# OSOceanAcoustics/echopype

Hardware: AMD Instinct MI355X
Metric: range-samples/sec through compute_Sv->compute_MVBS (higher is better)
Workload: dtype f64; 1 GPU; cfg5: EK60 CW 4x2000000x4096 in ping_time tiles, compute_Sv -> compute_MVBS(20s x 1m), Sv+MVBS out; tiles=8 x 250000 pings over 1 rank(s), route=compute_Sv -> compute_MVBS('1m','20s') per tile, collective=none at 1 rank, tile_streams=2

## Files before the change

### echopype_amd/csrc/fused_sv_mvbs.hip

```cpp
#include <hip/amd_detail/amd_hip_unsafe_atomics.h>

#include <cstdlib>
#include <type_traits>

#include "fast_math.h"
#include "sample_math.h"

namespace epa_fused {

constexpr int VEC = 4;
constexpr int kChunk = epa::kBlock * VEC;

struct Args {
  int P, S, n_tbins, n_rbins;
  double range_bin, inv_range_bin;
  double nspread, fill_value;
  unsigned guard, mask_range, skipna, closed_right;
  unsigned cnt_off, tab_off;
  unsigned long long* rmax_key;
  unsigned long long* rstat;
  int xcd_map;
  int flagged_only;
  const double* dscale;
  const double* doffset;
  void* depth_out;
};

__device__ __forceinline__ unsigned long long ordered_key(double v) {
  const unsigned long long b = __double_as_longlong(v);
  return (b >> 63) ? ~b : (b | 0x8000000000000000ull);
}

template <typename T>
__device__ __noinline__ T log10_slow(T x) {
  return epa::M<T>::log10(x);
}

template <typename T>
__device__ __forceinline__ void lds_add(T* p, T v) {
  unsafeAtomicAdd(p, v);
}

template <typename T>
struct Column {
  double sra;
  double blo, bhi;
  T nL;
  T acc_sum;
  int acc_rb;
  uint32_t acc_cnt;
  __device__ __forceinline__ void init() {
    sra = 0.0; blo = 1.0; bhi = 0.0; nL = epa::M<T>::nan(); acc_sum = (T)0; acc_rb = -1; acc_cnt = 0u;
  }
  __device__ __forceinline__ void flush(T* lsum, uint32_t* lcnt, uint32_t n_clean) {
    const uint32_t n = acc_cnt + n_clean;
    if (acc_rb >= 0 && n > 0u) {
      lds_add(lsum + acc_rb, acc_sum);
      atomicAdd(lcnt + acc_rb, n);
    }
  }
  __device__ __forceinline__ void rebin(double x, bool valid, double bin, double inv_bin, int n_rbins, T* lsum,
                                        uint32_t* lcnt, uint32_t n_clean) {
    const int rb = valid ? epa::range_bin_index(x, bin, inv_bin, n_rbins, false) : -1;
    if (rb != acc_rb) {
      flush(lsum, lcnt, n_clean);
      acc_rb = rb;
      acc_sum = (T)0;
      acc_cnt = 0u - n_clean;
    }
    blo = rb >= 0 ? (double)rb * bin : 1.0;
    bhi = rb >= 0 ? (double)(rb + 1) * bin : 0.0;
  }
};

__device__ __forceinline__ double lin_bins(double u, const double* __restrict__ tab) {
  constexpr double K256 = 85.04135922911648, Z = 0.0027076061740622863;
  constexpr double C1 = Z, C2 = Z * Z / 2.0, C3 = Z * Z * Z / 6.0;
  const double t = u * K256;
  const double m = __builtin_rint(t);
  const double r = fma(u, K256, -m);
  double p = fma(r, C3, C2);
  p = fma(p, r, C1);
  p = fma(p, r, 1.0);
  const int mi = __double2int_rz(m);
  return ldexp(p * tab[mi & 255], mi >> 8);
}
__device__ __forceinline__ float lin_bins(float u, const double*) { return ::exp10f(u * 0.1f); }

__device__ __forceinline__ double vmax_num(double a, double b) {
  double r;
  asm("v_max_f64 %0, %1, %2" : "=v"(r) : "v"(a), "v"(b));
  return r;
}
__device__ __forceinline__ float vmax_num(float a, float b) {
  float r;
  asm("v_max_f32 %0, %1, %2" : "=v"(r) : "v"(a), "v"(b));
  return r;
}
__device__ __forceinline__ double vmin_num(double a, double b) {
  double r;
  asm("v_min_f64 %0, %1, %2" : "=v"(r) : "v"(a), "v"(b));
  return r;
}

template <typename T, bool STATS>
__device__ __forceinline__ T process_sample(Column<T>& c, float raw, const epa::CoefRow& r, double r0v, T g, T a2,
                                            T A0v, T nL, T nspread, double bin, double inv_bin, int n_rbins,
                                            const double* tab, T* lsum, uint32_t* lcnt, double& xmax, double& xmin,
                                            unsigned& nnan, uint32_t n_clean) {
  const T NaN = epa::M<T>::nan();
  const double x = fma(c.sra, r.rb, r0v);
  if (STATS) {
    const double xq = fma((double)raw, 0.0, x);
    xmax = vmax_num(xmax, xq);
    xmin = vmin_num(xmin, xq);
    nnan += (unsigned)__builtin_popcountll(__ballot(raw != raw));
  }
  const double rtd = x - r.shift;
  const T rt = (T)rtd;
  const bool pos = rtd > 0.0;
  T s1 = fma(g, (T)raw, nL);
  if (pos & !(nL > -(T)__builtin_inf()))
    s1 = fma(g, (T)raw, nspread * (log10_slow<T>(rt) - log10_slow<T>((T)(r.ra * r.rb))));
  s1 = pos ? s1 : NaN;
  const T sv = s1 + fma(a2, rt, A0v);
  const T v = epa::lin_from_db_lean(sv, tab);
  const bool same = (x >= c.blo) & (x < c.bhi);
  if (!same) c.rebin(x, raw == raw, bin, inv_bin, n_rbins, lsum, lcnt, n_clean);
  c.acc_sum += vmax_num(v, (T)0);
  c.acc_cnt += v == v ? 1u : 0u;
  return sv;
}

template <typename T, bool STATS, bool WRITE_SV, int DEPTH>
__device__ __forceinline__ void process_pair(Column<T>& c0, Column<T>& c1, float2 in, bool clean, const epa::CoefRow& r,
                                             double r0v, T g, T a2, T A0v, T nL0, T nL1, T nspread, double bin,
                                             double inv_bin, int n_rbins, const double* tab, T* lsum, uint32_t* lcnt,
                                             T* __restrict__ sv_dst, double& xmax, double& xmin, unsigned& nnan,
                                             uint32_t n_clean, double& xfirst, double& xlast, T dsc, T dof,
                                             T* __restrict__ depth_dst, double sra0, double sra1) {
  const double e0 = fma(sra0, r.rb, r0v), e1 = fma(sra1, r.rb, r0v);
  const double rtd0 = e0 - r.shift, rtd1 = e1 - r.shift;
  T d0 = (T)0, d1 = (T)0;
  if (DEPTH) {
    d0 = epa::depth_of(dsc, dof, (T)e0);
    d1 = epa::depth_of(dsc, dof, (T)e1);
  }
  const double x0 = DEPTH ? (double)d0 : e0, x1 = DEPTH ? (double)d1 : e1;
  const T rt0 = (T)rtd0, rt1 = (T)rtd1;
  T s10 = fma(g, (T)in.x, nL0), s11 = fma(g, (T)in.y, nL1);
  if (!clean) {
    const T NaN = epa::M<T>::nan();
    const bool pos0 = rtd0 > 0.0, pos1 = rtd1 > 0.0;
    if (pos0 & !(nL0 > -(T)__builtin_inf()))
      s10 = fma(g, (T)in.x, nspread * (log10_slow<T>(rt0) - log10_slow<T>((T)(r.ra * r.rb))));
    if (pos1 & !(nL1 > -(T)__builtin_inf()))
      s11 = fma(g, (T)in.y, nspread * (log10_slow<T>(rt1) - log10_slow<T>((T)(r.ra * r.rb))));
    s10 = pos0 ? s10 : NaN;
    s11 = pos1 ? s11 : NaN;
    if (STATS) {
      const double xq0 = fma((double)in.x, 0.0, x0), xq1 = fma((double)in.y, 0.0, x1);
      xmax = vmax_num(vmax_num(xmax, xq0), xq1);
      xmin = vmin_num(vmin_num(xmin, xq0), xq1);
      nnan += (unsigned)__builtin_popcountll(__ballot(xq0 != xq0)) + (unsigned)__builtin_popcountll(__ballot(xq1 != xq1));
    }
    if (DEPTH == 2) {
      d0 = fma((T)in.x, (T)0, d0);
      d1 = fma((T)in.y, (T)0, d1);
    }
  }
  if (DEPTH == 2) epa::store_nt2(depth_dst, d0, d1);
  const T sv0 = s10 + fma(a2, rt0, A0v), sv1 = s11 + fma(a2, rt1, A0v);
  if (WRITE_SV) {
#ifndef EPA_PLAIN_STORES
    epa::store_nt2(sv_dst, sv0, sv1);
#else
    const T o[2] = {sv0, sv1};
    epa::store_vec<T, 2>(sv_dst, o);
#endif
  }
  T v0 = lin_bins(sv0, tab), v1 = lin_bins(sv1, tab);
  if (!clean) {
    if (__builtin_expect(__builtin_isinf(sv0), 0)) v0 = sv0 < (T)0 ? (T)0 : sv0;
    if (__builtin_expect(__builtin_isinf(sv1), 0)) v1 = sv1 < (T)0 ? (T)0 : sv1;
  }
  if (!((x0 >= c0.blo) & (x0 < c0.bhi))) c0.rebin(x0, in.x == in.x, bin, inv_bin, n_rbins, lsum, lcnt, n_clean);
  if (!((x1 >= c1.blo) & (x1 < c1.bhi))) c1.rebin(x1, in.y == in.y, bin, inv_bin, n_rbins, lsum, lcnt, n_clean);
  if (clean) {
    c0.acc_sum += v0;
    c1.acc_sum += v1;
  } else {
    c0.acc_sum += vmax_num(v0, (T)0);
    c1.acc_sum += vmax_num(v1, (T)0);
    c0.acc_cnt += v0 == v0 ? 1u : 0u;
    c1.acc_cnt += v1 == v1 ? 1u : 0u;
  }
  xfirst = x0;
  xlast = x1;
}

__device__ __forceinline__ bool not_finite(float x) { return __builtin_amdgcn_classf(x, 0x207); }

template <typename RawT>
struct PingLoad;
template <>
struct PingLoad<float> {
  float2 a, b;
  __device__ __forceinline__ PingLoad() : a(make_float2(0.f, 0.f)), b(make_float2(0.f, 0.f)) {}
  __device__ __forceinline__ void issue(const float* __restrict__ row, int sA, int sB, bool hasB, int, int) {
    a = *reinterpret_cast<const float2*>(row + sA);
    if (hasB) b = *reinterpret_cast<const float2*>(row + sB);
  }
  __device__ __forceinline__ void resolve(float2& A, float2& B, int, int, int, bool) const {
    A = a;
    B = b;
  }
};
template <>
struct PingLoad<int16_t> {
  unsigned a, b;
  __device__ __forceinline__ PingLoad() : a(0u), b(0u) {}
  __device__ __forceinline__ void issue(const int16_t* __restrict__ row, int sA, int sB, bool hasB, int, int) {
    a = *reinterpret_cast<const unsigned*>(row + sA);
    if (hasB) b = *reinterpret_cast<const unsigned*>(row + sB);
  }
  static __device__ __forceinline__ float2 unpack(unsigned w, int s, int n_valid) {
    constexpr float kIndex2Power = 0.011758984205624266f;
    const float nanv = __builtin_nanf("");
    const float x = (float)(short)(w & 0xffffu), y = (float)(short)(w >> 16);
    return make_float2(s < n_valid ? x * kIndex2Power : nanv, s + 1 < n_valid ? y * kIndex2Power : nanv);
  }
  static __device__ __forceinline__ float2 unpack_all(unsigned w) {
    constexpr float kIndex2Power = 0.011758984205624266f;
    return make_float2((float)(short)(w & 0xffffu) * kIndex2Power, (float)(short)(w >> 16) * kIndex2Power);
  }
  __device__ __forceinline__ void resolve(float2& A, float2& B, int sA, int sB, int nv, bool full) const {
    if (full) {
      A = unpack_all(a);
      B = unpack_all(b);
    } else {
      A = unpack(a, sA, nv);
      B = unpack(b, sB, nv);
    }
  }
};

#ifndef EPA_FUSED_MIN_WAVES
#define EPA_FUSED_MIN_WAVES 1
#endif
#ifndef EPA_FUSED_LEAN
#define EPA_FUSED_LEAN 1
#endif
__device__ __forceinline__ double uniform(double v) {
  return __hiloint2double(__builtin_amdgcn_readfirstlane(__double2hiint(v)), __builtin_amdgcn_readfirstlane(__double2loint(v)));
}

__device__ __forceinline__ bool finite_bits(double v) { return (__double2hiint(v) & 0x7ff00000) != 0x7ff00000; }

template <typename T, typename RawT, bool WRITE_SV, bool RMAX, int DEPTH>
__global__ __launch_bounds__(epa::kBlock, EPA_FUSED_MIN_WAVES > 4 ? EPA_FUSED_MIN_WAVES : 4) void fused_sv_mvbs_kernel(
    const RawT* __restrict__ raw, const int32_t* __restrict__ n_valid,
    const epa::CoefRow* __restrict__ coef,
    const int32_t* __restrict__ bin_start, T* __restrict__ sv_out, T* __restrict__ mvbs_out,
    T* __restrict__ sum_out, uint32_t* __restrict__ cnt_out, const double* __restrict__ dscale,
    const double* __restrict__ doffset, Args a) {
  extern __shared__ __attribute__((aligned(16))) unsigned char smem[];
  T* lsum = reinterpret_cast<T*>(smem);
  uint32_t* lcnt = reinterpret_cast<uint32_t*>(smem + a.cnt_off);
  const epa::MathTabs mt = epa::build_math_tabs(smem + a.tab_off);
  const double* tab = mt.exp2_tab;
  constexpr bool NL_LDS = RMAX || sizeof(T) == 8;
  __shared__ T col_nL[NL_LDS ? kChunk : 1];
  constexpr bool SRA_LDS = (RMAX || std::is_same<RawT, int16_t>::value) && sizeof(T) == 8;
  __shared__ double col_sra[SRA_LDS ? kChunk : 1];
  __shared__ unsigned long long wg_keys[2];
  __shared__ unsigned wg_nnan;
  if (RMAX && threadIdx.x == 0) {
    wg_keys[0] = 0ull;
    wg_keys[1] = ~0ull;
    wg_nnan = 0u;
  }

  const int c = blockIdx.y, tb = a.xcd_map ? epa::xcd_contiguous(blockIdx.x, a.n_tbins) : (int)blockIdx.x;
  const int S = a.S, n_rbins = a.n_rbins;
  const bool extra = tb == a.n_tbins;
  if (extra && !WRITE_SV) return;
  const int nseg = extra ? 2 : 1;
  for (int i = threadIdx.x; i < n_rbins; i += epa::kBlock) {
    lsum[i] = (T)0;
    lcnt[i] = 0u;
  }
  __syncthreads();

  const T nspread = (T)a.nspread;
  const double bin = a.range_bin, inv_bin = a.inv_range_bin;
  const epa::CoefRow* __restrict__ rowp0 = coef + (size_t)c * a.P;
  const RawT* __restrict__ raw_c = raw + (size_t)c * a.P * S;
  const int32_t* __restrict__ nv_c = n_valid ? n_valid + (size_t)c * a.P : nullptr;
  T* __restrict__ sv_c = WRITE_SV ? sv_out + (size_t)c * a.P * S : nullptr;
  T* __restrict__ dp_c = DEPTH == 2 ? reinterpret_cast<T*>(a.depth_out) + (size_t)c * a.P * S : nullptr;
  const double* __restrict__ dsc_c = DEPTH ? dscale + (size_t)c * a.P : nullptr;
  const double* __restrict__ dof_c = DEPTH ? doffset + (size_t)c * a.P : nullptr;
  const int wave = __builtin_amdgcn_readfirstlane((int)(threadIdx.x >> 6)), lane = threadIdx.x & 63;
  double xmax = -__builtin_inf(), xmin = __builtin_inf();
  unsigned nnan = 0u;

  for (int seg = 0; seg < nseg; ++seg) {
  const int pb = extra ? (seg == 0 ? 0 : bin_start[a.n_tbins]) : bin_start[tb];
  const int pe = extra ? (seg == 0 ? bin_start[0] : a.P) : bin_start[tb + 1];
  for (int chunk0 = 0; chunk0 < S; chunk0 += kChunk) {
    const int sA = chunk0 + wave * 256 + 2 * lane;
    const int sB = sA + 128;
    if (sA >= S) continue;
    const bool hasB = sB < S;
    Column<T> col[VEC];
#pragma unroll
    for (int j = 0; j < VEC; ++j) col[j].init();
    const int eA = wave * 256 + 2 * lane;
    if (NL_LDS) {
      col_nL[eA] = col_nL[eA + 1] = col_nL[eA + 128] = col_nL[eA + 129] = epa::M<T>::nan();
    }
    long long dcur = 0x7ff8dead00000001ll, racur = 0x7ff8dead00000002ll;
    uint32_t n_clean = 0u;
    bool plain = false;
    const int s4 = chunk0 + wave * 256 + 4 * lane;
    PingLoad<RawT> nxt;
    epa::CoefRow nxtR = rowp0[pb < pe ? pb : 0];
    double nxtDs = 1.0, nxtDo = 0.0;
    if (DEPTH) {
      nxtDs = uniform(dsc_c[pb < pe ? pb : 0]);
      nxtDo = uniform(dof_c[pb < pe ? pb : 0]);
    }
    int nxtNv = nv_c && pb < pe ? nv_c[pb] : S;
    if (pb < pe) nxt.issue(raw_c + (size_t)pb * S, sA, sB, hasB, s4, S);
    for (int p = pb; p < pe; ++p) {
      const epa::CoefRow r = nxtR;
      const double curDs = nxtDs, curDo = nxtDo;
      const size_t row_off = (size_t)p * S;
      const int nv = nxtNv;
      float2 inA, inB;
      const bool full = nv_c != nullptr && nv >= chunk0 + wave * 256 + 256;
      nxt.resolve(inA, inB, sA, sB, nv, full);
      if (p + 1 < pe) {
        nxtR = rowp0[p + 1];
        if (nv_c) nxtNv = nv_c[p + 1];
        if (DEPTH) {
          nxtDs = uniform(dsc_c[p + 1]);
          nxtDo = uniform(dof_c[p + 1]);
        }
        nxt.issue(raw_c + row_off + S, sA, sB, hasB, s4, S);
      }
      if (!((__double_as_longlong(r.d) == dcur) & (__double_as_longlong(r.ra) == racur))) {
        dcur = __double_as_longlong(r.d);
        racur = __double_as_longlong(r.ra);
        bool fin = true;
        for (int j = 0; j < VEC; ++j) {
          const double sj = (double)((j < 2 ? sA : sB) + (j & 1));
          const T nl = nspread * log10_slow<T>((T)(sj - r.d));
          if (NL_LDS) col_nL[eA + (j < 2 ? 0 : 128) + (j & 1)] = nl;
          else col[j].nL = nl;
          if (SRA_LDS) col_sra[eA + (j < 2 ? 0 : 128) + (j & 1)] = sj * r.ra;
          else col[j].sra = sj * r.ra;
          fin = fin & ((j >= 2 && !hasB) | (fabs(nl) < (T)__builtin_inf()));
        }
        plain = __ballot(!fin) == 0ull;
      }
      const T g = (T)r.g, a2 = (T)r.alpha2;
      T A0 = (T)r.A0;
      double r0v = r.r0;
      asm volatile("" : "+v"(A0), "+v"(r0v));
      bool clean = false;
#if EPA_FUSED_LEAN
      {
        const double xa = fma(SRA_LDS ? col_sra[eA] : col[0].sra, r.rb, r0v);
        bool bad = !(xa - r.shift > 0.0);
        if (!full) bad = bad | not_finite(inA.x) | not_finite(inA.y) | not_finite(inB.x) | not_finite(inB.y);
        bool kpos = (__double2hiint(r.ra) > 0) & (__double2hiint(r.rb) > 0) & finite_bits(r.g) & finite_bits(r.A0) &
                    finite_bits(r.alpha2);
        if (DEPTH) kpos = kpos & finite_bits(curDs) & finite_bits(curDo);
        clean = plain & kpos & (__ballot(bad) == 0ull);
      }
#endif
      const T dsc = (T)curDs, dof = (T)curDo;
      double xf, xl, xdummy;
      process_pair<T, RMAX, WRITE_SV, DEPTH>(col[0], col[1], inA, clean, r, r0v, g, a2, A0, NL_LDS ? col_nL[eA] : col[0].nL,
                                             NL_LDS ? col_nL[eA + 1] : col[1].nL, nspread, bin, inv_bin, n_rbins, tab, lsum,
                                             lcnt, WRITE_SV ? sv_c + row_off + sA : nullptr, xmax, xmin, nnan, n_clean, xf,
                                             xl, dsc, dof, DEPTH == 2 ? dp_c + row_off + sA : nullptr,
                                             SRA_LDS ? col_sra[eA] : col[0].sra, SRA_LDS ? col_sra[eA + 1] : col[1].sra);
      if (hasB)
        process_pair<T, RMAX, WRITE_SV, DEPTH>(col[2], col[3], inB, clean, r, r0v, g, a2, A0,
                                               NL_LDS ? col_nL[eA + 128] : col[2].nL, NL_LDS ? col_nL[eA + 129] : col[3].nL,
                                               nspread, bin, inv_bin, n_rbins, tab, lsum, lcnt,
                                               WRITE_SV ? sv_c + row_off + sB : nullptr, xmax, xmin, nnan, n_clean, xdummy,
                                               xl, dsc, dof, DEPTH == 2 ? dp_c + row_off + sB : nullptr,
                                               SRA_LDS ? col_sra[eA + 128] : col[2].sra,
                                               SRA_LDS ? col_sra[eA + 129] : col[3].sra);
      if (clean) {
        if (RMAX) {
          if (DEPTH) {
            xmin = vmin_num(vmin_num(xmin, xf), xl);
            xmax = vmax_num(vmax_num(xmax, xf), xl);
          } else {
            xmin = vmin_num(xmin, xf);
            xmax = vmax_num(xmax, xl);
          }
        }
        ++n_clean;
      }
    }
#pragma unroll
    for (int j = 0; j < VEC; ++j) col[j].flush(lsum, lcnt, n_clean);
  }
  }
  if (RMAX) {
#pragma unroll
    for (int o = 32; o > 0; o >>= 1) xmax = fmax(xmax, __shfl_down(xmax, o, 64));
#pragma unroll
    for (int o = 32; o > 0; o >>= 1) xmin = fmin(xmin, __shfl_down(xmin, o, 64));
    if (lane == 0) {
      if (xmax > -__builtin_inf()) atomicMax(&wg_keys[0], ordered_key(xmax));
      if (xmin < __builtin_inf()) atomicMin(&wg_keys[1], ordered_key(xmin));
      if (nnan > 0u) atomicAdd(&wg_nnan, nnan);
    }
    __syncthreads();
    if (threadIdx.x == 0) {
      const unsigned long long kmax = wg_keys[0], kmin = wg_keys[1];
      if (kmax != 0ull) atomicMax(a.rmax_key, kmax);
      if (a.rstat) {
        if (kmin != ~0ull) atomicMin(a.rstat, kmin);
        if (wg_nnan > 0u) atomicAdd(a.rstat + 1, (unsigned long long)wg_nnan);
      }
    }
  }
  if (extra) return;
  __syncthreads();
  const size_t cell0 = ((size_t)c * a.n_tbins + tb) * n_rbins;
  T* out = mvbs_out + cell0;
  T* gsum = sum_out ? sum_out + cell0 : nullptr;
  uint32_t* gcnt = cnt_out ? cnt_out + cell0 : nullptr;
  for (int i = threadIdx.x; i < n_rbins; i += epa::kBlock) {
    const uint32_t n = lcnt[i];
    const T s = lsum[i];
    out[i] = n > 0u ? (T)10 * epa::M<T>::log10(s / (T)n) : (T)a.fill_value;
    if (gsum) gsum[i] = s;
    if (gcnt) gcnt[i] = n;
  }
}

template <typename T, typename RawT>
int launch(Args& a, const RawT* raw, const int32_t* n_valid, const double* coef, const int32_t* bin_start,
           void* sv_out, void* mvbs_out, void* sum_out, uint32_t* cnt_out, int C, size_t lds_bytes,
           hipStream_t st) {
  const dim3 grid((unsigned)a.n_tbins + 1u, (unsigned)C);
  a.tab_off = (unsigned)((lds_bytes + 15) & ~(size_t)15);
  lds_bytes = a.tab_off + epa::kMathTabBytes;
  a.xcd_map = epa::xcd_map_enabled() ? 1 : 0;
#define EPA_FL(W, R) EPA_FLD(W, R, 0)
#define EPA_FLD(W, R, D)                                                                       \
  do {                                                                                         \
    auto kern = fused_sv_mvbs_kernel<T, RawT, W, R, D>;                                        \
    if (lds_bytes > 64 * 1024)                                                                 \
      EPA_CHECK_HIP(hipFuncSetAttribute(reinterpret_cast<const void*>(kern),                   \
                                        hipFuncAttributeMaxDynamicSharedMemorySize,            \
                                        (int)lds_bytes));                                      \
    hipLaunchKernelGGL(kern, grid, dim3(epa::kBlock), lds_bytes, st, raw, n_valid,             \
                       reinterpret_cast<const epa::CoefRow*>(coef), bin_start, (T*)sv_out,     \
                       (T*)mvbs_out, (T*)sum_out, cnt_out, a.dscale, a.doffset, a);            \
  } while (0)
  if (a.dscale) {
    if constexpr (std::is_same<RawT, float>::value) {
      if (a.depth_out) EPA_FLD(true, true, 2);
      else if (sv_out) EPA_FLD(true, true, 1);
      else EPA_FLD(false, true, 1);
    } else {
      epa::set_error("epa_sv_mvbs_fused_depth: float power samples only");
      return EPA_EUNSUPPORTED;
    }
  } else if (a.rmax_key) {
    if (sv_out) EPA_FL(true, true); else EPA_FL(false, true);
  } else {
    if (sv_out) EPA_FL(true, false); else EPA_FL(false, false);
  }
#undef EPA_FLD
#undef EPA_FL
  return epa::check_launch("fused_sv_mvbs_kernel");
}

__global__ __launch_bounds__(epa::kBlock) void selftest_lin_kernel(const double* __restrict__ u,
                                                                   double* __restrict__ out,
                                                                   size_t n) {
  __shared__ __attribute__((aligned(16))) unsigned char tabs[epa::kMathTabBytes];
  const epa::MathTabs mt = epa::build_math_tabs(tabs);
  __syncthreads();
  for (size_t i = (size_t)blockIdx.x * blockDim.x + threadIdx.x; i < n;
       i += (size_t)gridDim.x * blockDim.x)
    out[i] = epa::lin_from_db(u[i], mt.exp2_tab);
}

__global__ __launch_bounds__(epa::kBlock) void selftest_log_kernel(const double* __restrict__ x,
                                                                   double* __restrict__ out,
                                                                   size_t n) {
  __shared__ __attribute__((aligned(16))) unsigned char tabs[epa::kMathTabBytes];
  const epa::MathTabs mt = epa::build_math_tabs(tabs);
  __syncthreads();
  for (size_t i = (size_t)blockIdx.x * blockDim.x + threadIdx.x; i < n;
       i += (size_t)gridDim.x * blockDim.x)
    out[i] = epa::fast_log10(x[i], mt.log_tab);
}

__global__ __launch_bounds__(epa::kBlock) void selftest_log_inl_kernel(const double* __restrict__ x,
                                                                       double* __restrict__ out, size_t n) {
  __shared__ __attribute__((aligned(16))) unsigned char tabs[epa::kMathTabBytes];
  const epa::MathTabs mt = epa::build_math_tabs(tabs);
  __syncthreads();
  for (size_t i = (size_t)blockIdx.x * blockDim.x + threadIdx.x; i < n;
       i += (size_t)gridDim.x * blockDim.x)
    out[i] = epa::fast_log10_inl<false>(x[i], mt.log_tab);
}

template <typename T>
struct SvColumn {
  double sra, blo, bhi;
  T acc_sum;
  int acc_rb;
  uint32_t acc_cnt;
  __device__ __forceinline__ void init() { sra = 0.0; blo = 1.0; bhi = 0.0; acc_sum = (T)0; acc_rb = -1; acc_cnt = 0u; }
  __device__ __forceinline__ void flush(T* lsum, uint32_t* lcnt) {
    if (acc_rb >= 0 && acc_cnt > 0u) {
      lds_add(lsum + acc_rb, acc_sum);
      atomicAdd(lcnt + acc_rb, acc_cnt);
    }
  }
};

template <typename T, bool AS_STORED>
__device__ __forceinline__ void bin_sv_sample(SvColumn<T>& c, T sv, const epa::CoefRow& r, double bin, double inv_bin,
                                              int n_rbins, const double* tab, T* lsum, uint32_t* lcnt) {
  const double x0 = c.sra * r.rb + r.r0;
  const double x = AS_STORED ? (double)(T)x0 : x0;
  const T v = epa::lin_from_db(sv, tab);
  const bool same = (x >= c.blo) & (x < c.bhi);
  if (!same) {
    const int rb = (x == x) ? epa::range_bin_index(x, bin, inv_bin, n_rbins, false) : -1;
    if (rb != c.acc_rb) {
      c.flush(lsum, lcnt);
      c.acc_rb = rb;
      c.acc_sum = (T)0;
      c.acc_cnt = 0u;
    }
    c.blo = rb >= 0 ? (double)rb * bin : 1.0;
    c.bhi = rb >= 0 ? (double)(rb + 1) * bin : 0.0;
  }
  const bool take = (c.acc_rb >= 0) & (v == v);
  c.acc_sum += take ? v : (T)0;
  c.acc_cnt += take ? 1u : 0u;
}

constexpr int kFixedPings = 512;
template <typename T>
struct LeftMark;
template <>
struct LeftMark<double> {
  static constexpr unsigned long long kBits = 0x7ff8dead0c0ffee2ull;
};
template <>
struct LeftMark<float> {
  static constexpr unsigned kBits = 0x7fcdead2u;
};
__device__ __forceinline__ bool left_to_rows(const double* cell) {
  return *reinterpret_cast<const unsigned long long*>(cell) == LeftMark<double>::kBits;
}
__device__ __forceinline__ bool left_to_rows(const float* cell) {
  return *reinterpret_cast<const unsigned*>(cell) == LeftMark<float>::kBits;
}
__device__ __forceinline__ void mark_left(double* cell) {
  *reinterpret_cast<unsigned long long*>(cell) = LeftMark<double>::kBits;
}
__device__ __forceinline__ void mark_left(float* cell) { *reinterpret_cast<unsigned*>(cell) = LeftMark<float>::kBits; }

template <typename T, bool AS_STORED>
__global__ __launch_bounds__(epa::kBlock, sizeof(T) == 8 ? 6 : 8) void mvbs_of_sv_fixed_kernel(
    const T* __restrict__ sv, const epa::CoefRow* __restrict__ coef, const int32_t* __restrict__ bin_start,
    T* __restrict__ mvbs_out, T* __restrict__ sum_out, uint32_t* __restrict__ cnt_out, Args a) {
  typedef T T2 __attribute__((ext_vector_type(2)));
  extern __shared__ __attribute__((aligned(16))) unsigned char smem[];
  T* lsum = reinterpret_cast<T*>(smem);
  uint32_t* lcnt = reinterpret_cast<uint32_t*>(smem + a.cnt_off);
  const epa::MathTabs mt = epa::build_math_tabs(smem + a.tab_off);
  const double* tab = mt.exp2_tab;
  __shared__ int differs;
  __shared__ unsigned long long rb_lo_key, rb_hi_key;
  const int c = blockIdx.y, tb = a.xcd_map ? epa::xcd_contiguous(blockIdx.x, a.n_tbins) : (int)blockIdx.x;
  const int S = a.S, n_rbins = a.n_rbins;
  const int pb = bin_start[tb], pe = bin_start[tb + 1], np = pe - pb;
  const size_t cell0 = ((size_t)c * a.n_tbins + tb) * n_rbins;
  for (int i = threadIdx.x; i < n_rbins; i += epa::kBlock) {
    lsum[i] = (T)0;
    lcnt[i] = 0u;
  }
  if (threadIdx.x == 0) {
    differs = np > kFixedPings ? 1 : 0;
    rb_lo_key = ~0ull;
    rb_hi_key = 0ull;
  }
  __syncthreads();
  const epa::CoefRow* __restrict__ rowp0 = coef + (size_t)c * a.P;
  const epa::CoefRow r = rowp0[np > 0 ? pb : 0];
  for (int i = threadIdx.x; i < min(np, kFixedPings); i += epa::kBlock) {
    const epa::CoefRow ri = rowp0[pb + i];
    if (!((ri.ra == r.ra) & (ri.r0 == r.r0) & (ri.rb == ri.rb) & (ri.ra > 0.0))) differs = 1;
    atomicMin(&rb_lo_key, ordered_key(ri.rb));
    atomicMax(&rb_hi_key, ordered_key(ri.rb));
  }
  __syncthreads();
  if (differs) {
    if (threadIdx.x == 0) mark_left(mvbs_out + cell0);
    return;
  }
  auto unkey = [](unsigned long long k) {
    return __longlong_as_double((long long)((k >> 63) ? (k & 0x7fffffffffffffffull) : ~k));
  };
  const double rb_lo = unkey(rb_lo_key), rb_hi = unkey(rb_hi_key);
  const double bin = a.range_bin, inv_bin = a.inv_range_bin;
  const T* __restrict__ sv_c = sv + (size_t)c * a.P * S;
  const int wave = threadIdx.x >> 6, lane = threadIdx.x & 63;
  auto range_of = [&](int sx, double rb) {
    const double x0 = ((double)sx * r.ra) * rb + r.r0;
    return AS_STORED ? (double)(T)x0 : x0;
  };
  for (int chunk0 = 0; chunk0 < S; chunk0 += kChunk) {
    const int sA = chunk0 + wave * 256 + 2 * lane;
    const int sB = sA + 128;
    if (sA >= S) continue;
    const bool hasB = sB < S;
    int rbin[VEC];
    T acc_sum[VEC];
    uint32_t acc_cnt[VEC];
    unsigned fixed = 0;
#pragma unroll
    for (int j = 0; j < VEC; ++j) {
      const int sx = (j < 2 ? sA : sB) + (j & 1);
      const int b_lo = epa::range_bin_index(range_of(sx, rb_lo), bin, inv_bin, n_rbins, false);
      const int b_hi = epa::range_bin_index(range_of(sx, rb_hi), bin, inv_bin, n_rbins, false);
      rbin[j] = b_lo;
      if (b_lo == b_hi) fixed |= 1u << j;
      acc_sum[j] = (T)0;
      acc_cnt[j] = 0u;
    }
    T2 nA0 = {(T)0, (T)0}, nB0 = nA0, nA1 = nA0, nB1 = nA0;
    if (np > 0) {
      nA0 = *reinterpret_cast<const T2*>(sv_c + (size_t)pb * S + sA);
      if (hasB) nB0 = *reinterpret_cast<const T2*>(sv_c + (size_t)pb * S + sB);
    }
    if (np > 1) {
      nA1 = *reinterpret_cast<const T2*>(sv_c + (size_t)(pb + 1) * S + sA);
      if (hasB) nB1 = *reinterpret_cast<const T2*>(sv_c + (size_t)(pb + 1) * S + sB);
    }
    for (int p = pb; p < pe; ++p) {
      const T2 inA = nA0, inB = nB0;
      nA0 = nA1;
      nB0 = nB1;
      if (p + 2 < pe) {
        const T* nx = sv_c + (size_t)(p + 2) * S;
        nA1 = *reinterpret_cast<const T2*>(nx + sA);
        if (hasB) nB1 = *reinterpret_cast<const T2*>(nx + sB);
      }
      const T in[VEC] = {inA.x, inA.y, inB.x, inB.y};
#pragma unroll
      for (int j = 0; j < VEC; ++j) {
        if (j >= 2 && !hasB) break;
        const T v = epa::lin_from_db_lean(in[j], tab);
        acc_sum[j] += vmax_num(v, (T)0);
        acc_cnt[j] += v == v ? 1u : 0u;
      }
    }
#pragma unroll
    for (int j = 0; j < VEC; ++j) {
      if (((fixed >> j) & 1u) != 0u && rbin[j] >= 0 && acc_cnt[j] > 0u) {
        lds_add(lsum + rbin[j], acc_sum[j]);
        atomicAdd(lcnt + rbin[j], acc_cnt[j]);
      }
    }
    const unsigned loose = (~fixed) & (hasB ? 0xfu : 0x3u);
    if (__ballot(loose != 0u) != 0ull) {
      const int nact = (int)__popcll(__ballot(true));
#pragma unroll 1
      for (int j = 0; j < VEC; ++j) {
        unsigned long long todo = __ballot(((loose >> j) & 1u) != 0u);
        while (todo != 0ull) {
          const int src = __ffsll((long long)todo) - 1;
          todo &= todo - 1ull;
          const int sx = chunk0 + wave * 256 + 2 * src + (j < 2 ? 0 : 128) + (j & 1);
          for (int p = pb + lane; p < pe; p += nact) {
            const T v = epa::lin_from_db_lean(sv_c[(size_t)p * S + sx], tab);
            const double x = range_of(sx, rowp0[p].rb);
            const int rb = epa::range_bin_index(x, bin, inv_bin, n_rbins, false);
            if ((rb >= 0) & (v == v)) {
              lds_add(lsum + rb, v);
              atomicAdd(lcnt + rb, 1u);
            }
          }
        }
      }
    }
  }
  __syncthreads();
  T* out = mvbs_out + cell0;
  T* gsum = sum_out ? sum_out + cell0 : nullptr;
  uint32_t* gcnt = cnt_out ? cnt_out + cell0 : nullptr;
  for (int i = threadIdx.x; i < n_rbins; i += epa::kBlock) {
    const uint32_t n = lcnt[i];
    const T s = lsum[i];
    out[i] = n > 0u ? (T)10 * epa::M<T>::log10(s / (T)n) : (T)a.fill_value;
    if (gsum) gsum[i] = s;
    if (gcnt) gcnt[i] = n;
  }
}

template <typename T, bool AS_STORED>
__global__ __launch_bounds__(epa::kBlock, EPA_FUSED_MIN_WAVES) void mvbs_of_sv_rows_kernel(
    const T* __restrict__ sv, const epa::CoefRow* __restrict__ coef, const int32_t* __restrict__ bin_start,
    T* __restrict__ mvbs_out, T* __restrict__ sum_out, uint32_t* __restrict__ cnt_out, Args a) {
  typedef T T2 __attribute__((ext_vector_type(2)));
  extern __shared__ __attribute__((aligned(16))) unsigned char smem[];
  T* lsum = reinterpret_cast<T*>(smem);
  uint32_t* lcnt = reinterpret_cast<uint32_t*>(smem + a.cnt_off);
  const epa::MathTabs mt = epa::build_math_tabs(smem + a.tab_off);
  const double* tab = mt.exp2_tab;
  const int c = blockIdx.y, tb = a.xcd_map ? epa::xcd_contiguous(blockIdx.x, a.n_tbins) : (int)blockIdx.x;
  const int S = a.S, n_rbins = a.n_rbins;
  if (a.flagged_only && !left_to_rows(mvbs_out + ((size_t)c * a.n_tbins + tb) * n_rbins)) return;
// ... 172 lines not shown
```

Baseline: 453.3 billion range-samples/s.

## Prefetch multiple ping rows ahead via register queue with cross-chunk priming

Replaces the single-row-ahead raw load with a D-deep register queue of outstanding ping-row loads. An unrolled steady-state loop issues each refill D rows ahead, and the queue for the next chunk or segment is primed before the current one flushes. This is meant to hide global load latency in this memory-bound kernel. It also drops the cached bin bounds from Column in favour of recomputing them from acc_rb, which saves registers but adds a multiply per check. Sv stores switch to plain vector stores by default instead of nontemporal ones. The deeper queue raises register pressure and may lower occupancy.

```diff
diff --git a/echopype_amd/csrc/fused_sv_mvbs.hip b/echopype_amd/csrc/fused_sv_mvbs.hip
--- a/echopype_amd/csrc/fused_sv_mvbs.hip
+++ b/echopype_amd/csrc/fused_sv_mvbs.hip
@@ -4,6 +4,7 @@
 #include <type_traits>
 
 #include "fast_math.h"
+#include "rows_queue.h"
 #include "sample_math.h"
 
 namespace epa_fused {
@@ -44,13 +45,15 @@
 template <typename T>
 struct Column {
   double sra;
-  double blo, bhi;
   T nL;
   T acc_sum;
   int acc_rb;
   uint32_t acc_cnt;
   __device__ __forceinline__ void init() {
-    sra = 0.0; blo = 1.0; bhi = 0.0; nL = epa::M<T>::nan(); acc_sum = (T)0; acc_rb = -1; acc_cnt = 0u;
+    sra = 0.0; nL = epa::M<T>::nan(); acc_sum = (T)0; acc_rb = -1; acc_cnt = 0u;
+  }
+  __device__ __forceinline__ bool in_bin(double x, double bin) const {
+    return (acc_rb >= 0) & (x >= (double)acc_rb * bin) & (x < (double)(acc_rb + 1) * bin);
   }
   __device__ __forceinline__ void flush(T* lsum, uint32_t* lcnt, uint32_t n_clean) {
     const uint32_t n = acc_cnt + n_clean;
@@ -68,8 +71,6 @@
       acc_sum = (T)0;
       acc_cnt = 0u - n_clean;
     }
-    blo = rb >= 0 ? (double)rb * bin : 1.0;
-    bhi = rb >= 0 ? (double)(rb + 1) * bin : 0.0;
   }
 };
 
@@ -101,6 +102,16 @@
   double r;
   asm("v_min_f64 %0, %1, %2" : "=v"(r) : "v"(a), "v"(b));
   return r;
+}
+
+#ifndef EPA_FUSED_MEM_FLAVOUR
+#define EPA_FUSED_MEM_FLAVOUR 2
+#endif
+constexpr bool kNtRawLoads = (EPA_FUSED_MEM_FLAVOUR & 1) != 0;
+constexpr bool kPlainSvStores = (EPA_FUSED_MEM_FLAVOUR & 2) != 0;
+template <typename V>
+__device__ __forceinline__ V load_raw(const V* p) {
+  return kNtRawLoads ? __builtin_nontemporal_load(p) : *p;
 }
 
 template <typename T, bool STATS>
@@ -125,7 +136,7 @@
   s1 = pos ? s1 : NaN;
   const T sv = s1 + fma(a2, rt, A0v);
   const T v = epa::lin_from_db_lean(sv, tab);
-  const bool same = (x >= c.blo) & (x < c.bhi);
+  const bool same = c.in_bin(x, bin);
   if (!same) c.rebin(x, raw == raw, bin, inv_bin, n_rbins, lsum, lcnt, n_clean);
   c.acc_sum += vmax_num(v, (T)0);
   c.acc_cnt += v == v ? 1u : 0u;
@@ -172,20 +183,20 @@
   if (DEPTH == 2) epa::store_nt2(depth_dst, d0, d1);
   const T sv0 = s10 + fma(a2, rt0, A0v), sv1 = s11 + fma(a2, rt1, A0v);
   if (WRITE_SV) {
-#ifndef EPA_PLAIN_STORES
-    epa::store_nt2(sv_dst, sv0, sv1);
-#else
-    const T o[2] = {sv0, sv1};
-    epa::store_vec<T, 2>(sv_dst, o);
-#endif
+    if (kPlainSvStores) {
+      typedef T T2 __attribute__((ext_vector_type(2)));
+      *reinterpret_cast<T2*>(sv_dst) = T2{sv0, sv1};
+    } else {
+      epa::store_nt2(sv_dst, sv0, sv1);
+    }
   }
   T v0 = lin_bins(sv0, tab), v1 = lin_bins(sv1, tab);
   if (!clean) {
     if (__builtin_expect(__builtin_isinf(sv0), 0)) v0 = sv0 < (T)0 ? (T)0 : sv0;
     if (__builtin_expect(__builtin_isinf(sv1), 0)) v1 = sv1 < (T)0 ? (T)0 : sv1;
   }
-  if (!((x0 >= c0.blo) & (x0 < c0.bhi))) c0.rebin(x0, in.x == in.x, bin, inv_bin, n_rbins, lsum, lcnt, n_clean);
-  if (!((x1 >= c1.blo) & (x1 < c1.bhi))) c1.rebin(x1, in.y == in.y, bin, inv_bin, n_rbins, lsum, lcnt, n_clean);
+  if (!c0.in_bin(x0, bin)) c0.rebin(x0, in.x == in.x, bin, inv_bin, n_rbins, lsum, lcnt, n_clean);
+  if (!c1.in_bin(x1, bin)) c1.rebin(x1, in.y == in.y, bin, inv_bin, n_rbins, lsum, lcnt, n_clean);
   if (clean) {
     c0.acc_sum += v0;
     c1.acc_sum += v1;
@@ -203,13 +214,14 @@
 
 template <typename RawT>
 struct PingLoad;
+__device__ __forceinline__ float2 to_float2(epa::epa_f2 v) { return make_float2(v.x, v.y); }
 template <>
 struct PingLoad<float> {
   float2 a, b;
   __device__ __forceinline__ PingLoad() : a(make_float2(0.f, 0.f)), b(make_float2(0.f, 0.f)) {}
-  __device__ __forceinline__ void issue(const float* __restrict__ row, int sA, int sB, bool hasB, int, int) {
-    a = *reinterpret_cast<const float2*>(row + sA);
-    if (hasB) b = *reinterpret_cast<const float2*>(row + sB);
+  __device__ __forceinline__ void issue(const float* __restrict__ row, int sA, int sBl) {
+    a = to_float2(load_raw(reinterpret_cast<const epa::epa_f2*>(row + sA)));
+    b = to_float2(load_raw(reinterpret_cast<const epa::epa_f2*>(row + sBl)));
   }
   __device__ __forceinline__ void resolve(float2& A, float2& B, int, int, int, bool) const {
     A = a;
@@ -220,9 +232,9 @@
 struct PingLoad<int16_t> {
   unsigned a, b;
   __device__ __forceinline__ PingLoad() : a(0u), b(0u) {}
-  __device__ __forceinline__ void issue(const int16_t* __restrict__ row, int sA, int sB, bool hasB, int, int) {
-    a = *reinterpret_cast<const unsigned*>(row + sA);
-    if (hasB) b = *reinterpret_cast<const unsigned*>(row + sB);
+  __device__ __forceinline__ void issue(const int16_t* __restrict__ row, int sA, int sBl) {
+    a = load_raw(reinterpret_cast<const unsigned*>(row + sA));
+    b = load_raw(reinterpret_cast<const unsigned*>(row + sBl));
   }
   static __device__ __forceinline__ float2 unpack(unsigned w, int s, int n_valid) {
     constexpr float kIndex2Power = 0.011758984205624266f;
@@ -256,6 +268,19 @@
 }
 
 __device__ __forceinline__ bool finite_bits(double v) { return (__double2hiint(v) & 0x7ff00000) != 0x7ff00000; }
+
+constexpr int kMaxRowsAhead = 6;
+template <typename T, typename RawT, bool WRITE_SV, bool RMAX, int DEPTH>
+constexpr int rows_ahead() {
+#ifdef EPA_FUSED_ROWS_AHEAD
+  return EPA_FUSED_ROWS_AHEAD;
+#else
+  if (sizeof(T) == 4) return kMaxRowsAhead;
+  if (!WRITE_SV) return 4;
+  if (std::is_same<RawT, int16_t>::value) return RMAX ? 1 : 4;
+  return DEPTH == 2 ? 4 : (RMAX ? 2 : 3);
+#endif
+}
 
 template <typename T, typename RawT, bool WRITE_SV, bool RMAX, int DEPTH>
 __global__ __launch_bounds__(epa::kBlock, EPA_FUSED_MIN_WAVES > 4 ? EPA_FUSED_MIN_WAVES : 4) void fused_sv_mvbs_kernel(
@@ -305,14 +330,29 @@
   double xmax = -__builtin_inf(), xmin = __builtin_inf();
   unsigned nnan = 0u;
 
+  constexpr int D = rows_ahead<T, RawT, WRITE_SV, RMAX, DEPTH>();
+  PingLoad<RawT> q[D];
+  auto prime = [&](int pb_, int pe_, int sA_) {
+    if (epa::rows_queue_prime(pb_, pe_, D) == D) {
+      const int sBl = sA_ + 128 < S ? sA_ + 128 : sA_;
+#pragma unroll
+      for (int k = 0; k < D; ++k) q[k].issue(raw_c + (size_t)(pb_ + k) * S, sA_, sBl);
+    }
+  };
+  auto seg_begin = [&](int seg) { return extra ? (seg == 0 ? 0 : bin_start[a.n_tbins]) : bin_start[tb]; };
+  auto seg_end = [&](int seg) { return extra ? (seg == 0 ? bin_start[0] : a.P) : bin_start[tb + 1]; };
+  bool primed = false;
+
   for (int seg = 0; seg < nseg; ++seg) {
-  const int pb = extra ? (seg == 0 ? 0 : bin_start[a.n_tbins]) : bin_start[tb];
-  const int pe = extra ? (seg == 0 ? bin_start[0] : a.P) : bin_start[tb + 1];
+  const int pb = seg_begin(seg), pe = seg_end(seg);
   for (int chunk0 = 0; chunk0 < S; chunk0 += kChunk) {
     const int sA = chunk0 + wave * 256 + 2 * lane;
     const int sB = sA + 128;
     if (sA >= S) continue;
     const bool hasB = sB < S;
+    const int sBl = hasB ? sB : sA;
+    if (!primed) prime(pb, pe, sA);
+    primed = false;
     Column<T> col[VEC];
 #pragma unroll
     for (int j = 0; j < VEC; ++j) col[j].init();
@@ -323,8 +363,6 @@
     long long dcur = 0x7ff8dead00000001ll, racur = 0x7ff8dead00000002ll;
     uint32_t n_clean = 0u;
     bool plain = false;
-    const int s4 = chunk0 + wave * 256 + 4 * lane;
-    PingLoad<RawT> nxt;
     epa::CoefRow nxtR = rowp0[pb < pe ? pb : 0];
     double nxtDs = 1.0, nxtDo = 0.0;
     if (DEPTH) {
@@ -332,15 +370,16 @@
       nxtDo = uniform(dof_c[pb < pe ? pb : 0]);
     }
     int nxtNv = nv_c && pb < pe ? nv_c[pb] : S;
-    if (pb < pe) nxt.issue(raw_c + (size_t)pb * S, sA, sB, hasB, s4, S);
-    for (int p = pb; p < pe; ++p) {
+    const bool queued = epa::rows_queue_prime(pb, pe, D) == D;
+    auto ping = [&](const PingLoad<RawT>& cur, PingLoad<RawT>& fill, const int p, auto steady)
+                    __attribute__((always_inline)) {
       const epa::CoefRow r = nxtR;
       const double curDs = nxtDs, curDo = nxtDo;
       const size_t row_off = (size_t)p * S;
       const int nv = nxtNv;
       float2 inA, inB;
       const bool full = nv_c != nullptr && nv >= chunk0 + wave * 256 + 256;
-      nxt.resolve(inA, inB, sA, sB, nv, full);
+      cur.resolve(inA, inB, sA, sB, nv, full);
       if (p + 1 < pe) {
         nxtR = rowp0[p + 1];
         if (nv_c) nxtNv = nv_c[p + 1];
@@ -348,7 +387,6 @@
           nxtDs = uniform(dsc_c[p + 1]);
           nxtDo = uniform(dof_c[p + 1]);
         }
-        nxt.issue(raw_c + row_off + S, sA, sB, hasB, s4, S);
       }
       if (!((__double_as_longlong(r.d) == dcur) & (__double_as_longlong(r.ra) == racur))) {
         dcur = __double_as_longlong(r.d);
@@ -407,6 +445,32 @@
           }
         }
         ++n_clean;
+      }
+      if (decltype(steady)::value) {
+        fill.issue(raw_c + (size_t)(p + D) * S, sA, sBl);
+      } else {
+        const int pn = queued ? epa::rows_queue_next(p, pe, D) : -1;
+        if (pn >= 0) fill.issue(raw_c + (size_t)pn * S, sA, sBl);
+      }
+    };
+    int p0 = pb;
+    for (; epa::rows_queue_steady(p0, pe, D); p0 += D) {
+#pragma unroll
+      for (int k = 0; k < D; ++k) ping(q[k], q[k], p0 + k, std::true_type());
+    }
+    for (int p = p0; p < pe; ++p) {
+      if (!queued) q[0].issue(raw_c + (size_t)p * S, sA, sBl);
+      const PingLoad<RawT> cur = q[0];
+#pragma unroll
+      for (int k = 0; k + 1 < D; ++k) q[k] = q[k + 1];
+      ping(cur, q[D - 1], p, std::false_type());
+    }
+    {
+      const bool last = chunk0 + kChunk >= S;
+      const int nseg_ = last ? seg + 1 : seg, nsA = last ? sA - chunk0 : sA + kChunk;
+      if (nseg_ < nseg && nsA < S) {
+        prime(last ? seg_begin(nseg_) : pb, last ? seg_end(nseg_) : pe, nsA);
+        primed = true;
       }
     }
 #pragma unroll
diff --git a/echopype_amd/csrc/rows_queue.h b/echopype_amd/csrc/rows_queue.h
--- /dev/null
+++ b/echopype_amd/csrc/rows_queue.h
@@ -0,0 +1,17 @@
+#pragma once
+
+#if defined(__HIPCC__) || defined(__CUDACC__)
+#define EPA_ROWS_HD __host__ __device__
+#else
+#define EPA_ROWS_HD
+#endif
+
+namespace epa {
+
+EPA_ROWS_HD inline int rows_queue_prime(int pb, int pe, int D) { return pe - pb >= D ? D : 0; }
+
+EPA_ROWS_HD inline bool rows_queue_steady(int p0, int pe, int D) { return pe - p0 >= 2 * D; }
+
+EPA_ROWS_HD inline int rows_queue_next(int p, int pe, int D) { return pe - p > D ? p + D : -1; }
+
+}
```

Result: slower. 439.6 billion range-samples/s (-3.0%).

## Add fixed-range fast path kernel for fused Sv+MVBS with fallback flagging

Applied to the files above, without the earlier changes.

Adds a specialised fused kernel for time bins whose calibration coefficients are uniform across pings. In that case each sample column maps to a fixed range bin, so values accumulate in registers and are added to shared memory once per column instead of once per sample. Bins that fail the uniformity check are marked with a sentinel, and the general kernel then runs only on those flagged bins. The cost is an extra kernel launch, a coefficient-scan prologue, and more code paths. The new path is on by default for float raw input and can be disabled through an environment variable.

```diff
diff --git a/echopype_amd/csrc/fused_sv_mvbs.hip b/echopype_amd/csrc/fused_sv_mvbs.hip
--- a/echopype_amd/csrc/fused_sv_mvbs.hip
+++ b/echopype_amd/csrc/fused_sv_mvbs.hip
@@ -245,6 +245,28 @@
   }
 };
 
+constexpr int kFixedPings = 512;
+template <typename T>
+struct LeftMark;
+template <>
+struct LeftMark<double> {
+  static constexpr unsigned long long kBits = 0x7ff8dead0c0ffee2ull;
+};
+template <>
+struct LeftMark<float> {
+  static constexpr unsigned kBits = 0x7fcdead2u;
+};
+__device__ __forceinline__ bool left_to_rows(const double* cell) {
+  return *reinterpret_cast<const unsigned long long*>(cell) == LeftMark<double>::kBits;
+}
+__device__ __forceinline__ bool left_to_rows(const float* cell) {
+  return *reinterpret_cast<const unsigned*>(cell) == LeftMark<float>::kBits;
+}
+__device__ __forceinline__ void mark_left(double* cell) {
+  *reinterpret_cast<unsigned long long*>(cell) = LeftMark<double>::kBits;
+}
+__device__ __forceinline__ void mark_left(float* cell) { *reinterpret_cast<unsigned*>(cell) = LeftMark<float>::kBits; }
+
 #ifndef EPA_FUSED_MIN_WAVES
 #define EPA_FUSED_MIN_WAVES 1
 #endif
@@ -264,6 +286,10 @@
     const int32_t* __restrict__ bin_start, T* __restrict__ sv_out, T* __restrict__ mvbs_out,
     T* __restrict__ sum_out, uint32_t* __restrict__ cnt_out, const double* __restrict__ dscale,
     const double* __restrict__ doffset, Args a) {
+  if (a.flagged_only && (int)blockIdx.x != a.n_tbins &&
+      !left_to_rows(mvbs_out + ((size_t)blockIdx.y * a.n_tbins +
+                                (a.xcd_map ? epa::xcd_contiguous(blockIdx.x, a.n_tbins) : (int)blockIdx.x)) * a.n_rbins))
+    return;
   extern __shared__ __attribute__((aligned(16))) unsigned char smem[];
   T* lsum = reinterpret_cast<T*>(smem);
   uint32_t* lcnt = reinterpret_cast<uint32_t*>(smem + a.cnt_off);
@@ -448,6 +474,264 @@
   }
 }
 
+template <typename T, bool STATS, bool WRITE_SV>
+__device__ __forceinline__ void fixed_pair(T& sum0, T& sum1, uint32_t* cnt, float2 in, bool clean,
+                                           const epa::CoefRow& r, double r0v, T g, T a2, T A0v, T nL0, T nL1, 
+                                           const double* tab, T* __restrict__ sv_dst, double& xmax, double& xmin,
+                                           unsigned& nnan, double& xfirst, double& xlast, double sra0, double sra1) {
+  const double x0 = fma(sra0, r.rb, r0v), x1 = fma(sra1, r.rb, r0v);
+  const double rtd0 = x0 - r.shift, rtd1 = x1 - r.shift;
+  const T rt0 = (T)rtd0, rt1 = (T)rtd1;
+  T s10 = fma(g, (T)in.x, nL0), s11 = fma(g, (T)in.y, nL1);
+  bool res0 = false, res1 = false;
+  if (!clean) {
+    const T NaN = epa::M<T>::nan();
+    const bool pos0 = rtd0 > 0.0, pos1 = rtd1 > 0.0;
+    res0 = pos0 & !(nL0 > -(T)__builtin_inf());
+    res1 = pos1 & !(nL1 > -(T)__builtin_inf());
+    s10 = pos0 ? s10 : NaN;
+    s11 = pos1 ? s11 : NaN;
+    if (STATS) {
+      const double xq0 = fma((double)in.x, 0.0, x0), xq1 = fma((double)in.y, 0.0, x1);
+      xmax = vmax_num(vmax_num(xmax, xq0), xq1);
+      xmin = vmin_num(vmin_num(xmin, xq0), xq1);
+      nnan += (unsigned)__builtin_popcountll(__ballot(xq0 != xq0)) + (unsigned)__builtin_popcountll(__ballot(xq1 != xq1));
+    }
+  }
+  const T sv0 = s10 + fma(a2, rt0, A0v), sv1 = s11 + fma(a2, rt1, A0v);
+  if (WRITE_SV) {
+    if (clean || !(res0 | res1)) {
+      epa::store_nt2(sv_dst, sv0, sv1);
+    } else {
+      if (!res0) sv_dst[0] = sv0;
+      if (!res1) sv_dst[1] = sv1;
+    }
+  }
+  T v0 = lin_bins(sv0, tab), v1 = lin_bins(sv1, tab);
+  if (clean) {
+    sum0 += v0;
+    sum1 += v1;
+  } else {
+    if (__builtin_expect(__builtin_isinf(sv0), 0)) v0 = sv0 < (T)0 ? (T)0 : sv0;
+    if (__builtin_expect(__builtin_isinf(sv1), 0)) v1 = sv1 < (T)0 ? (T)0 : sv1;
+    sum0 += vmax_num(v0, (T)0);
+    sum1 += vmax_num(v1, (T)0);
+    if (v0 == v0) atomicAdd(cnt, 1u);
+    if (v1 == v1) atomicAdd(cnt + 1, 1u);
+  }
+  xfirst = x0;
+  xlast = x1;
+}
+
+#ifndef EPA_FIXED_W64
+#define EPA_FIXED_W64 6
+#endif
+#ifndef EPA_FIXED_W64S
+#define EPA_FIXED_W64S 5
+#endif
+#ifndef EPA_FIXED_W32
+#define EPA_FIXED_W32 6
+#endif
+template <typename T, bool WRITE_SV, bool RMAX>
+__global__ __launch_bounds__(epa::kBlock, sizeof(T) == 8 ? (RMAX ? EPA_FIXED_W64S : EPA_FIXED_W64) : EPA_FIXED_W32) void fused_sv_mvbs_fixed_kernel(
+    const float* __restrict__ raw, const epa::CoefRow* __restrict__ coef, const int32_t* __restrict__ bin_start,
+    T* __restrict__ sv_out, T* __restrict__ mvbs_out, T* __restrict__ sum_out, uint32_t* __restrict__ cnt_out, Args a) {
+  extern __shared__ __attribute__((aligned(16))) unsigned char smem[];
+  T* lsum = reinterpret_cast<T*>(smem);
+  uint32_t* lcnt = reinterpret_cast<uint32_t*>(smem + a.cnt_off);
+  const epa::MathTabs mt = epa::build_math_tabs(smem + a.tab_off);
+  const double* tab = mt.exp2_tab;
+  __shared__ uint32_t col_cnt[kChunk];
+  __shared__ int differs;
+  __shared__ unsigned long long rb_lo_key, rb_hi_key;
+  __shared__ unsigned long long wg_keys[2];
+  __shared__ unsigned wg_nnan;
+  const int c = blockIdx.y, tb = a.xcd_map ? epa::xcd_contiguous(blockIdx.x, a.n_tbins) : (int)blockIdx.x;
+  const int S = a.S, n_rbins = a.n_rbins;
+  const int pb = bin_start[tb], pe = bin_start[tb + 1], np = pe - pb;
+  const size_t cell0 = ((size_t)c * a.n_tbins + tb) * n_rbins;
+  for (int i = threadIdx.x; i < n_rbins; i += epa::kBlock) {
+    lsum[i] = (T)0;
+    lcnt[i] = 0u;
+  }
+  if (threadIdx.x == 0) {
+    differs = np > kFixedPings ? 1 : 0;
+    rb_lo_key = ~0ull;
+    rb_hi_key = 0ull;
+    wg_keys[0] = 0ull;
+    wg_keys[1] = ~0ull;
+    wg_nnan = 0u;
+  }
+  __syncthreads();
+  const epa::CoefRow* __restrict__ rowp0 = coef + (size_t)c * a.P;
+  const epa::CoefRow r = rowp0[np > 0 ? pb : 0];
+  for (int i = threadIdx.x; i < min(np, kFixedPings); i += epa::kBlock) {
+    const epa::CoefRow ri = rowp0[pb + i];
+    if (!((ri.ra == r.ra) & (ri.r0 == r.r0) & (ri.d == r.d) & (ri.ra > 0.0) & (ri.ra < __builtin_inf()) & (ri.rb > 0.0) &
+          (ri.rb < __builtin_inf())))
+      differs = 1;
+    atomicMin(&rb_lo_key, ordered_key(ri.rb));
+    atomicMax(&rb_hi_key, ordered_key(ri.rb));
+  }
+  __syncthreads();
+  if (differs) {
+    if (threadIdx.x == 0) mark_left(mvbs_out + cell0);
+    return;
+  }
+  auto unkey = [](unsigned long long k) {
+    return __longlong_as_double((long long)((k >> 63) ? (k & 0x7fffffffffffffffull) : ~k));
+  };
+  const double rb_lo = unkey(rb_lo_key), rb_hi = unkey(rb_hi_key);
+  const T nspread = (T)a.nspread;
+  const double bin = a.range_bin, inv_bin = a.inv_range_bin;
+  const float* __restrict__ raw_c = raw + (size_t)c * a.P * S;
+  T* __restrict__ sv_c = WRITE_SV ? sv_out + (size_t)c * a.P * S : nullptr;
+  const int wave = __builtin_amdgcn_readfirstlane((int)(threadIdx.x >> 6)), lane = threadIdx.x & 63;
+  double xmax = -__builtin_inf(), xmin = __builtin_inf();
+  unsigned nnan = 0u;
+
+  for (int chunk0 = 0; np > 0 && chunk0 < S; chunk0 += kChunk) {
+    const int sA = chunk0 + wave * 256 + 2 * lane;
+    const int sB = sA + 128;
+    if (sA >= S) continue;
+    const bool hasB = sB < S;
+    T nL[VEC], acc_sum[VEC];
+    double sra[VEC];
+    const int eA = wave * 256 + 2 * lane;
+    bool fin = true;
+#pragma unroll
+    for (int j = 0; j < VEC; ++j) {
+      const double sj = (double)((j < 2 ? sA : sB) + (j & 1));
+      nL[j] = nspread * log10_slow<T>((T)(sj - r.d));
+      sra[j] = sj * r.ra;
+      fin = fin & ((j >= 2 && !hasB) | (fabs(nL[j]) < (T)__builtin_inf()));
+      acc_sum[j] = (T)0;
+      col_cnt[eA + (j < 2 ? 0 : 128) + (j & 1)] = 0u;
+    }
+    const bool plain = __ballot(!fin) == 0ull;
+    uint32_t n_clean = 0u;
+    PingLoad<float> nxt;
+    epa::CoefRow nxtR = rowp0[pb];
+    nxt.issue(raw_c + (size_t)pb * S, sA, sB, hasB, 0, S);
+    for (int p = pb; p < pe; ++p) {
+      const epa::CoefRow rp = nxtR;
+      const size_t row_off = (size_t)p * S;
+      float2 inA, inB;
+      nxt.resolve(inA, inB, sA, sB, S, false);
+      if (p + 1 < pe) {
+        nxtR = rowp0[p + 1];
+        nxt.issue(raw_c + row_off + S, sA, sB, hasB, 0, S);
+      }
+      const T g = (T)rp.g, a2 = (T)rp.alpha2;
+      T A0 = (T)rp.A0;
+      double r0v = rp.r0;
+      asm volatile("" : "+v"(A0), "+v"(r0v));
+      const double xa = fma(sra[0], rp.rb, r0v);
+      const bool bad = !(xa - rp.shift > 0.0) | not_finite(inA.x) | not_finite(inA.y) | not_finite(inB.x) | not_finite(inB.y);
+      const bool kpos = (__double2hiint(rp.ra) > 0) & (__double2hiint(rp.rb) > 0) & finite_bits(rp.g) & finite_bits(rp.A0) &
+                        finite_bits(rp.alpha2);
+      const bool clean = plain & kpos & (__ballot(bad) == 0ull);
+      double xf, xl, xdummy;
+      fixed_pair<T, RMAX, WRITE_SV>(acc_sum[0], acc_sum[1], col_cnt + eA, inA, clean, rp, r0v, g, a2, A0, nL[0],
+                                    nL[1], tab, WRITE_SV ? sv_c + row_off + sA : nullptr, xmax, xmin, nnan, xf, xl,
+                                    sra[0], sra[1]);
+      if (hasB)
+        fixed_pair<T, RMAX, WRITE_SV>(acc_sum[2], acc_sum[3], col_cnt + eA + 128, inB, clean, rp, r0v, g, a2, A0, nL[2],
+                                      nL[3], tab, WRITE_SV ? sv_c + row_off + sB : nullptr, xmax, xmin, nnan,
+                                      xdummy, xl, sra[2], sra[3]);
+      if (clean) {
+        if (RMAX) {
+          xmin = vmin_num(xmin, xf);
+          xmax = vmax_num(xmax, xl);
+        }
+        ++n_clean;
+      }
+    }
+    unsigned loose = 0u;
+#pragma unroll
+    for (int j = 0; j < VEC; ++j) {
+      if (j >= 2 && !hasB) break;
+      const double x_lo = fma(sra[j], rb_lo, r.r0), x_hi = fma(sra[j], rb_hi, r.r0);
+      const int b_lo = epa::range_bin_index(x_lo, bin, inv_bin, n_rbins, false);
+      const int b_hi = epa::range_bin_index(x_hi, bin, inv_bin, n_rbins, false);
+      const bool fixed = b_lo == b_hi && (b_lo >= 0 || !((x_lo < 0.0) & (x_hi > 0.0))) && nL[j] > -(T)__builtin_inf();
+      const uint32_t n = col_cnt[eA + (j < 2 ? 0 : 128) + (j & 1)] + n_clean;
+      if (!fixed) {
+        loose |= 1u << j;
+      } else if (b_lo >= 0 && n > 0u) {
+        lds_add(lsum + b_lo, acc_sum[j]);
+        atomicAdd(lcnt + b_lo, n);
+      }
+    }
+    if (__ballot(loose != 0u) != 0ull) {
+      const int nact = (int)__popcll(__ballot(true));
+      const T NaN = epa::M<T>::nan();
+#pragma unroll 1
+      for (int j = 0; j < VEC; ++j) {
+        unsigned long long todo = __ballot(((loose >> j) & 1u) != 0u);
+        while (todo != 0ull) {
+          const int src = __ffsll((long long)todo) - 1;
+          todo &= todo - 1ull;
+          const int sx = chunk0 + wave * 256 + 2 * src + (j < 2 ? 0 : 128) + (j & 1);
+          const double sxd = (double)sx, sra_x = sxd * r.ra;
+          const T nl = nspread * log10_slow<T>((T)(sxd - r.d));
+          for (int p = pb + lane; p < pe; p += nact) {
+            const epa::CoefRow rp = rowp0[p];
+            const float rawv = raw_c[(size_t)p * S + sx];
+            const double x = fma(sra_x, rp.rb, rp.r0);
+            const double rtd = x - rp.shift;
+            const T rt = (T)rtd, g = (T)rp.g;
+            const bool pos = rtd > 0.0;
+            T s1 = fma(g, (T)rawv, nl);
+            if (pos & !(nl > -(T)__builtin_inf()))
+              s1 = fma(g, (T)rawv, nspread * (log10_slow<T>(rt) - log10_slow<T>((T)(rp.ra * rp.rb))));
+            s1 = pos ? s1 : NaN;
+            const T sv = s1 + fma((T)rp.alpha2, rt, (T)rp.A0);
+            if (WRITE_SV && pos && !(nl > -(T)__builtin_inf())) sv_c[(size_t)p * S + sx] = sv;
+            const T v = epa::lin_from_db_lean(sv, tab);
+            const int rb = epa::range_bin_index(x, bin, inv_bin, n_rbins, false);
+            if ((rb >= 0) & (v == v)) {
+              lds_add(lsum + rb, v);
+              atomicAdd(lcnt + rb, 1u);
+            }
+          }
+        }
+      }
+    }
+  }
+  if (RMAX) {
+#pragma unroll
+    for (int o = 32; o > 0; o >>= 1) xmax = fmax(xmax, __shfl_down(xmax, o, 64));
+#pragma unroll
+    for (int o = 32; o > 0; o >>= 1) xmin = fmin(xmin, __shfl_down(xmin, o, 64));
+    if (lane == 0) {
+      if (xmax > -__builtin_inf()) atomicMax(&wg_keys[0], ordered_key(xmax));
+      if (xmin < __builtin_inf()) atomicMin(&wg_keys[1], ordered_key(xmin));
+      if (nnan > 0u) atomicAdd(&wg_nnan, nnan);
+    }
+    __syncthreads();
+    if (threadIdx.x == 0) {
+      const unsigned long long kmax = wg_keys[0], kmin = wg_keys[1];
+      if (kmax != 0ull) atomicMax(a.rmax_key, kmax);
+      if (a.rstat) {
+        if (kmin != ~0ull) atomicMin(a.rstat, kmin);
+        if (wg_nnan > 0u) atomicAdd(a.rstat + 1, (unsigned long long)wg_nnan);
+      }
+    }
+  }
+  __syncthreads();
+  T* out = mvbs_out + cell0;
+  T* gsum = sum_out ? sum_out + cell0 : nullptr;
+  uint32_t* gcnt = cnt_out ? cnt_out + cell0 : nullptr;
+  for (int i = threadIdx.x; i < n_rbins; i += epa::kBlock) {
+    const uint32_t n = lcnt[i];
+    const T s = lsum[i];
+    out[i] = n > 0u ? (T)10 * epa::M<T>::log10(s / (T)n) : (T)a.fill_value;
+    if (gsum) gsum[i] = s;
+    if (gcnt) gcnt[i] = n;
+  }
+}
+
 template <typename T, typename RawT>
 int launch(Args& a, const RawT* raw, const int32_t* n_valid, const double* coef, const int32_t* bin_start,
            void* sv_out, void* mvbs_out, void* sum_out, uint32_t* cnt_out, int C, size_t lds_bytes,
@@ -468,6 +752,30 @@
                        reinterpret_cast<const epa::CoefRow*>(coef), bin_start, (T*)sv_out,     \
                        (T*)mvbs_out, (T*)sum_out, cnt_out, a.dscale, a.doffset, a);            \
   } while (0)
+  a.flagged_only = 0;
+  if constexpr (std::is_same<RawT, float>::value) {
+    const char* knob = getenv("EPA_FUSED_FIXED");
+    if (!a.dscale && a.n_tbins > 0 && a.n_rbins > 0 && !(knob && knob[0] == '0' && knob[1] == 0)) {
+#define EPA_FX(W, R)                                                                                          \
+  do {                                                                                                        \
+    auto kern = fused_sv_mvbs_fixed_kernel<T, W, R>;                                                          \
+    if (lds_bytes > 64 * 1024)                                                                                \
+      EPA_CHECK_HIP(hipFuncSetAttribute(reinterpret_cast<const void*>(kern),                                  \
+                                        hipFuncAttributeMaxDynamicSharedMemorySize, (int)lds_bytes));         \
+    hipLaunchKernelGGL(kern, dim3((unsigned)a.n_tbins, (unsigned)C), dim3(epa::kBlock), lds_bytes, st, raw,   \
+                       reinterpret_cast<const epa::CoefRow*>(coef), bin_start, (T*)sv_out, (T*)mvbs_out,      \
+                       (T*)sum_out, cnt_out, a);                                                              \
+  } while (0)
+      if (a.rmax_key) {
+        if (sv_out) EPA_FX(true, true); else EPA_FX(false, true);
+      } else {
+        if (sv_out) EPA_FX(true, false); else EPA_FX(false, false);
+      }
+#undef EPA_FX
+      if (int rc = epa::check_launch("fused_sv_mvbs_fixed_kernel")) return rc;
+      a.flagged_only = 1;
+    }
+  }
   if (a.dscale) {
     if constexpr (std::is_same<RawT, float>::value) {
       if (a.depth_out) EPA_FLD(true, true, 2);
@@ -556,28 +864,6 @@
   c.acc_sum += take ? v : (T)0;
   c.acc_cnt += take ? 1u : 0u;
 }
-
-constexpr int kFixedPings = 512;
-template <typename T>
-struct LeftMark;
-template <>
-struct LeftMark<double> {
-  static constexpr unsigned long long kBits = 0x7ff8dead0c0ffee2ull;
-};
-template <>
-struct LeftMark<float> {
-  static constexpr unsigned kBits = 0x7fcdead2u;
-};
-__device__ __forceinline__ bool left_to_rows(const double* cell) {
-  return *reinterpret_cast<const unsigned long long*>(cell) == LeftMark<double>::kBits;
-}
-__device__ __forceinline__ bool left_to_rows(const float* cell) {
-  return *reinterpret_cast<const unsigned*>(cell) == LeftMark<float>::kBits;
-}
-__device__ __forceinline__ void mark_left(double* cell) {
-  *reinterpret_cast<unsigned long long*>(cell) = LeftMark<double>::kBits;
-}
-__device__ __forceinline__ void mark_left(float* cell) { *reinterpret_cast<unsigned*>(cell) = LeftMark<float>::kBits; }
 
 template <typename T, bool AS_STORED>
 __global__ __launch_bounds__(epa::kBlock, sizeof(T) == 8 ? 6 : 8) void mvbs_of_sv_fixed_kernel(
```

Measured after the change: 496.3 billion range-samples/s before, 491.1 billion range-samples/s after. 0.99x the previous value.
